# Carlos310197/Fast-Point-Cloud-Registration-with-GPUs

Measured on AMD Instinct MI355X. Metric: ICP iterations/sec + NN HBM GB/s (% roofline), hall cloud, higher is better.
Workload: dtype f32

## Files before the change

fast-point-cloud-registration-with-gpus_amd/csrc/icp_device_sparse.h:

```cpp
#pragma once
#include "icp_device.h"

namespace icp {

template <bool HIER> struct SpHit { using type = unsigned short; };
template <> struct SpHit<true> { using type = int; };

constexpr bool SP_XY_EARLY_OUT = false;

template <bool PERM, int S>
__device__ __forceinline__ void scan_hit_half(const float* sb, int ch, const f2 px, const f2 py, const f2 pz, float& best, int& bj, float (&bq)[3])
{
    constexpr int C = 8;
    const float *qxp = sb + 8, *qyp = sb + 16, *qzp = sb + 24;
    const float4 qxa = *reinterpret_cast<const float4*>(qxp), qxb = *reinterpret_cast<const float4*>(qxp + 4);
    const float4 qya = *reinterpret_cast<const float4*>(qyp), qyb = *reinterpret_cast<const float4*>(qyp + 4);
    const float4 qza = *reinterpret_cast<const float4*>(qzp), qzb = *reinterpret_cast<const float4*>(qzp + 4);
    f2 d[C / 2];
    {
        f2 ax, ay, az;
        ax = pk_sub_sel<S>(f2{qxa.x, qxa.y}, px); ay = pk_sub_sel<S>(f2{qya.x, qya.y}, py); az = pk_sub_sel<S>(f2{qza.x, qza.y}, pz); d[0] = (ax * ax + ay * ay) + az * az;
        ax = pk_sub_sel<S>(f2{qxa.z, qxa.w}, px); ay = pk_sub_sel<S>(f2{qya.z, qya.w}, py); az = pk_sub_sel<S>(f2{qza.z, qza.w}, pz); d[1] = (ax * ax + ay * ay) + az * az;
        ax = pk_sub_sel<S>(f2{qxb.x, qxb.y}, px); ay = pk_sub_sel<S>(f2{qyb.x, qyb.y}, py); az = pk_sub_sel<S>(f2{qzb.x, qzb.y}, pz); d[2] = (ax * ax + ay * ay) + az * az;
        ax = pk_sub_sel<S>(f2{qxb.z, qxb.w}, px); ay = pk_sub_sel<S>(f2{qyb.z, qyb.w}, py); az = pk_sub_sel<S>(f2{qzb.z, qzb.w}, pz); d[3] = (ax * ax + ay * ay) + az * az;
    }
    float c0 = fmin_(fmin_(d[0].x, d[0].y), fmin_(d[1].x, d[1].y));
    c0 = fmin_(c0, fmin_(fmin_(d[2].x, d[2].y), fmin_(d[3].x, d[3].y)));
    auto dk = [&](int k) { return (k & 1) ? d[k >> 1].y : d[k >> 1].x; };
    if constexpr (PERM) {
        const bool cand = c0 <= best;
        if (__builtin_amdgcn_ballot_w64(cand) != 0ull) {
            const int* qo = reinterpret_cast<const int*>(sb + 32);
            int o0 = 0x7fffffff, k0 = 0;
#pragma unroll
            for (int kk = C - 1; kk >= 0; --kk) {
                const int oj = qo[kk];
                const bool e0 = (dk(kk) == c0) & (oj < o0);
                o0 = e0 ? oj : o0; k0 = e0 ? kk : k0;
            }
            const bool take = cand & ((c0 < best) | (bj < 0) | (o0 < bj));
            best = take ? c0 : best;
            bj = take ? o0 : bj;
            if (take) { bq[0] = qxp[k0]; bq[1] = qyp[k0]; bq[2] = qzp[k0]; }
        }
    } else {
        const bool take = (c0 < best) | ((c0 == best) & (ch < (bj >> 3)));
        if (__builtin_amdgcn_ballot_w64(take) != 0ull) {
            int k0 = C - 1;
#pragma unroll
            for (int kk = C - 2; kk >= 0; --kk) k0 = (dk(kk) == c0) ? kk : k0;
            best = take ? c0 : best;
            bj = take ? ch * C + k0 : bj;
            if (take) { bq[0] = qxp[k0]; bq[1] = qyp[k0]; bq[2] = qzp[k0]; }
        }
    }
}

template <bool PERM, bool HALVES = false>
__device__ __forceinline__ int scan_hit(const float* sb, int ch, const f2 px, const f2 py, const f2 pz, float (&best)[2], int (&bj)[2],
                                        float (&bq)[2][3])
{
    constexpr int C = 8;
    {
        if constexpr (HALVES) {
            const f2 gx = px - f2{__builtin_amdgcn_fmed3f(px.x, sb[0], sb[3]), __builtin_amdgcn_fmed3f(px.y, sb[0], sb[3])};
            const f2 gy = py - f2{__builtin_amdgcn_fmed3f(py.x, sb[1], sb[4]), __builtin_amdgcn_fmed3f(py.y, sb[1], sb[4])};
            const f2 gz = pz - f2{__builtin_amdgcn_fmed3f(pz.x, sb[2], sb[5]), __builtin_amdgcn_fmed3f(pz.y, sb[2], sb[5])};
            f2 L = (gx * gx + gy * gy) + gz * gz;
            L = L * f2{0.99999905f, 0.99999905f};
            const unsigned long long m0 = __builtin_amdgcn_ballot_w64(L.x <= best[0]), m1 = __builtin_amdgcn_ballot_w64(L.y <= best[1]);
            if ((m0 | m1) == 0ull) return 0;
            if (m1 == 0ull) { scan_hit_half<PERM, 0>(sb, ch, px, py, pz, best[0], bj[0], bq[0]); return 2; }
            if (m0 == 0ull) { scan_hit_half<PERM, 1>(sb, ch, px, py, pz, best[1], bj[1], bq[1]); return 2; }
        } else {
        const f2 pxa[1] = {px}, pya[1] = {py}, pza[1] = {pz};
        if (__builtin_amdgcn_ballot_w64(box_may_improve<1, true>(sb[0], sb[1], sb[2], sb[3], sb[4], sb[5], pxa, pya, pza, best)) == 0ull) return 0;
        }
    }
    const float *qxp = sb + 8, *qyp = sb + 16, *qzp = sb + 24;
    f2 d[C];
    float mxy0 = inf_<float>(), mxy1 = inf_<float>();
#pragma unroll
    for (int kk = 0; kk < C; kk += 4) {
        const float4 qx4 = *reinterpret_cast<const float4*>(qxp + kk);
        const float4 qy4 = *reinterpret_cast<const float4*>(qyp + kk);
        const f2 qxa = f2{qx4.x, qx4.y}, qxb = f2{qx4.z, qx4.w};
        const f2 qya = f2{qy4.x, qy4.y}, qyb = f2{qy4.z, qy4.w};
        f2 ax, ay;
        ax = pk_sub_bcast<0>(qxa, px); ay = pk_sub_bcast<0>(qya, py);
        d[kk + 0] = ax * ax + ay * ay;
        ax = pk_sub_bcast<1>(qxa, px); ay = pk_sub_bcast<1>(qya, py);
        d[kk + 1] = ax * ax + ay * ay;
        ax = pk_sub_bcast<0>(qxb, px); ay = pk_sub_bcast<0>(qyb, py);
        d[kk + 2] = ax * ax + ay * ay;
        ax = pk_sub_bcast<1>(qxb, px); ay = pk_sub_bcast<1>(qyb, py);
        d[kk + 3] = ax * ax + ay * ay;
        if constexpr (SP_XY_EARLY_OUT) {
            mxy0 = fmin_(fmin_(mxy0, d[kk].x), d[kk + 1].x);
            mxy0 = fmin_(fmin_(mxy0, d[kk + 2].x), d[kk + 3].x);
            mxy1 = fmin_(fmin_(mxy1, d[kk].y), d[kk + 1].y);
            mxy1 = fmin_(fmin_(mxy1, d[kk + 2].y), d[kk + 3].y);
        }
    }
    if constexpr (SP_XY_EARLY_OUT) {
        if (__builtin_amdgcn_ballot_w64((mxy0 <= best[0]) | (mxy1 <= best[1])) == 0ull) return 1;
    }
    float c0 = inf_<float>(), c1 = inf_<float>();
#pragma unroll
    for (int kk = 0; kk < C; kk += 4) {
        const float4 qz4 = *reinterpret_cast<const float4*>(qzp + kk);
        const f2 qza = f2{qz4.x, qz4.y}, qzb = f2{qz4.z, qz4.w};
        f2 az;
        az = pk_sub_bcast<0>(qza, pz); d[kk + 0] = d[kk + 0] + az * az;
        az = pk_sub_bcast<1>(qza, pz); d[kk + 1] = d[kk + 1] + az * az;
        az = pk_sub_bcast<0>(qzb, pz); d[kk + 2] = d[kk + 2] + az * az;
        az = pk_sub_bcast<1>(qzb, pz); d[kk + 3] = d[kk + 3] + az * az;
        c0 = fmin_(fmin_(c0, d[kk].x), d[kk + 1].x);
        c0 = fmin_(fmin_(c0, d[kk + 2].x), d[kk + 3].x);
        c1 = fmin_(fmin_(c1, d[kk].y), d[kk + 1].y);
        c1 = fmin_(fmin_(c1, d[kk + 2].y), d[kk + 3].y);
    }
    if constexpr (PERM) {
        const bool cand0 = c0 <= best[0], cand1 = c1 <= best[1];
        if (__builtin_amdgcn_ballot_w64(cand0 | cand1) != 0ull) {
            const int* qo = reinterpret_cast<const int*>(sb + 32);
            int o0 = 0x7fffffff, o1 = 0x7fffffff, k0 = 0, k1 = 0;
// ... 283 lines not shown
```

fast-point-cloud-registration-with-gpus_amd/csrc/icp_k_sparse.hip:

```cpp
#include "icp_device_sparse.h"
#include <math.h>
#include <stdlib.h>
#include <cstring>

namespace icp {


template <int TAIL, bool DIAG, bool PERM, bool HIER = false, int NWS = SP_NW>
__global__ __launch_bounds__(NWS * 64, NWS == 16 ? 1 : 4) void nn_match_sparse(const float* __restrict__ P, int n_pad,
                                                              const float* __restrict__ Q, int m_pad, int seg_len,
                                                              int round_passes, float* __restrict__ part_d,
                                                              int32_t* __restrict__ part_idx, RT<float> rt_arg, NNFuse fuse,
                                                              NNTail tail)
{
    constexpr int STG = PERM ? 40 : 32;
    constexpr int SMAX = NWS != 16 ? 1024 : 2048;
    constexpr int HITS_BYTES = SP_HCAP * 4, MQ_BYTES = NWS * 128 * 4;
    constexpr int SUPER_BYTES = HIER ? 2 * NWS * 64 * 4 : 0;
    constexpr int MKEY_OFF = 3 * SMAX * 4 > HITS_BYTES + SUPER_BYTES ? 3 * SMAX * 4 : HITS_BYTES + SUPER_BYTES;
    constexpr int OVL_BYTES = NWS != 16 ? MKEY_OFF + 128 * 8 : HITS_BYTES + 2 * SP_NW * 128 * 4;
    constexpr int TR_BYTES = TAIL ? ((TAIL == 2 ? 28 : 18) * 65 + 64) * 8 : 0;
    static_assert(TR_BYTES <= HITS_BYTES, "the tail's transpose buffer overlays the hit list");
    constexpr int HB = HIER ? 16 : 8;
    constexpr int STAGE_OFF = OVL_BYTES + 128 * 4 + 16, STAGE_BYTES = NWS * HB * STG * 4;
// ... 61 lines not shown
                const unsigned int sums[4] = {s01 & 0xffffu, s01 >> 16, s23 & 0xffffu, s23 >> 16};
                T = share_pick(T0, Tmin, sums, gridDim.x);
            }
            unsigned int S = parts_for(T);
            int v = (int)S;
#pragma unroll
            for (int o = 1; o < 64; o <<= 1) { const int u = __shfl_up(v, o, 64); v += lane >= o ? u : 0; }
            if (lane == 63) role[4 + NWS + w] = v;
            __syncthreads();
            int base = 0;
#pragma unroll
            for (int k = 0; k < NWS; ++k) base += k < w ? role[4 + NWS + k] : 0;
            int all = 0;
#pragma unroll
            for (int k = 0; k < NWS; ++k) all += role[4 + NWS + k];
            const bool fits = all <= (int)gridDim.x;
            const int excl = fits ? base + v - (int)S : t;
            if (!fits) S = t < R ? 1u : 0u;
            if (t < R && (int)blockIdx.x >= excl && (int)blockIdx.x < excl + (int)S) { role[0] = t; role[1] = (int)blockIdx.x - excl; role[2] = (int)S; if constexpr (DIAG) { role[3] = (int)h; role[4] = (int)T; } }
            __syncthreads();
            if (role[0] < 0) return;
            if (t == 0) role[5] = 0;
        }
    }
    if constexpr (HIER && TAIL != 0) {
        if (fuse.row_order != nullptr) {
            int bpos = (int)blockIdx.x;
            {
                const int sh = fuse.xcd_shift, span = 8 << sh;
                if (sh > 0 && bpos < ((int)gridDim.x / span) * span) {
                    const int x = bpos & 7, i = bpos >> 3;
                    bpos = ((((i >> sh) << 3) + x) << sh) + (i & ((1 << sh) - 1));
                }
            }
            const int ro = fuse.row_order[bpos];
            if (ro < 0) return;
            if (threadIdx.x == 0) {
                role[0] = ro & ((1 << NN_ROLE_ROW_BITS) - 1);
                role[1] = (ro >> NN_ROLE_ROW_BITS) & ((1 << NN_ROLE_PART_BITS) - 1);
                role[2] = 1 << ((ro >> (NN_ROLE_ROW_BITS + NN_ROLE_PART_BITS)) & 7);
            }
            __syncthreads();
        }
    }
    unsigned int hsum = 0;
    const int ibase = SP_ROW * 128 + lane;
    int pi[2];
#pragma unroll
    for (int t = 0; t < 2; ++t) pi[t] = fuse.p_perm ? fuse.p_perm[ibase + t * 64] : ibase + t * 64;
    float* stage = reinterpret_cast<float*>(lds_raw + STAGE_OFF) + w * (HB * STG);
    float* msg = reinterpret_cast<float*>(lds_raw + MSG_OFF);
    float (*seedq)[128] = reinterpret_cast<float (*)[128]>(lds_raw + SEED_OFF);
    float (*mq)[NWS][128] = reinterpret_cast<float (*)[NWS][128]>(lds_raw + MQ_OFF);
    int phase_pass_ = 0;
    constexpr int phase_nw_ = NWS;
    constexpr bool phase_diag_ = DIAG;
    ICP_PHASE(0)
    const int q0 = SP_SHARED ? 0 : (int)blockIdx.y * seg_len;
    const int c_lo = q0 / 8, c_hi = min(q0 + seg_len, m_pad) / 8;
    bool real[2], sok[2];
    float sq[2][3];
    const bool from_slots = fuse.slot_state != nullptr && fuse.slot_valid != 0;
#pragma unroll
    for (int t = 0; t < 2; ++t) {
        real[t] = ibase + t * 64 < fuse.n;
        sok[t] = false;
        sq[t][0] = sq[t][1] = sq[t][2] = 0.f;
        if (from_slots) {
            const float* ss = fuse.slot_state + 3 * (size_t)n_pad + (ibase + t * 64);
            sq[t][0] = ss[0]; sq[t][1] = ss[(size_t)n_pad]; sq[t][2] = ss[2 * (size_t)n_pad];
            sok[t] = real[t];
        } else {
            const int i = fresh(pi[t]);
            int j = !real[t] ? -1 : fuse.seed_idx ? fuse.seed_idx[i] : (int)(((long long)i * fuse.m) / fuse.n);
            sok[t] = (unsigned)j < (unsigned)fuse.m;
            j = sok[t] ? j : 0;
            const float* Qg = fuse.Q_gather;
            sq[t][0] = Qg[j]; sq[t][1] = Qg[(size_t)m_pad + j]; sq[t][2] = Qg[2 * (size_t)m_pad + j];
        }
    }
    f2 px, py, pz;
    if (from_slots) {
        const float* ss = fuse.slot_state + (fuse.slot_flip ? 6 * (size_t)n_pad : 0) + ibase;
        px = f2{ss[0], ss[64]};
        py = f2{ss[(size_t)n_pad], ss[(size_t)n_pad + 64]};
        pz = f2{ss[2 * (size_t)n_pad], ss[2 * (size_t)n_pad + 64]};
    } else {
        px = f2{P[pi[0]], P[pi[1]]};
        py = f2{P[(size_t)n_pad + pi[0]], P[(size_t)n_pad + pi[1]]};
        pz = f2{P[2 * (size_t)n_pad + pi[0]], P[2 * (size_t)n_pad + pi[1]]};
    }
    float4 pb0 = float4{0.f, 0.f, 0.f, 0.f}, pb1 = pb0;
    float4 (*boxc)[2][64] = reinterpret_cast<float4 (*)[2][64]>(lds_raw + BOXC_OFF) + w * PRE;
    if constexpr (HIER) {
        const int n2_all = ((m_pad >> 3) + 63) >> 6;
        const int t_lo = c_lo >> 12, t_hi = ((((c_hi + 63) >> 6)) + 63) >> 6;
        const int tidx = t_lo + w * 64 + lane;
        const float4* bp = reinterpret_cast<const float4*>(fuse.boxes + (size_t)m_pad + ((size_t)n2_all + (size_t)(tidx < t_hi ? tidx : t_lo)) * 8);
        pb0 = bp[0];
        pb1 = bp[1];
    } else {
        static_assert(PRE == 2, "two passes are fetched together");
        const int tparts = SP_SHARED ? SP_PARTS : 1, tpart = SP_SHARED ? SP_PART : 0;
        const int ca = c_lo + (w * 64 + lane) * tparts + tpart, cb = ca + NWS * 64 * tparts;
        const float4* bpa = reinterpret_cast<const float4*>(fuse.boxes + (size_t)(ca < c_hi ? ca : 0) * 8);
        const float4* bpb = reinterpret_cast<const float4*>(fuse.boxes + (size_t)(cb < c_hi ? cb : 0) * 8);
        const float4 a0 = bpa[0], a1 = bpa[1], b0 = bpb[0], b1 = bpb[1];
        boxc[0][0][lane] = a0; boxc[0][1][lane] = a1;
        boxc[1][0][lane] = b0; boxc[1][1][lane] = b1;
    }
    unsigned int wk_find = 0, wk_upper = 0, wk_hit[3] = {0, 0, 0}, wk_samp = 0;
    bool spec_valid = false;
    float* spst = reinterpret_cast<float*>(lds_raw + SPST_OFF) + w * 8;
    for (int pass = 0;; ++pass) {
    phase_pass_ = pass;
    double err_row = 0.0;
    RT<float> rt = rt_arg;
    int cmd = fuse.apply ? ICP_CMD_TRANSFORM_MATCH : ICP_CMD_MATCH;
    double row_tag = tail.tag;
    unsigned int row_tag_lo = tail.tag_lo;
    const bool have_seeds = pass > 0 || fuse.seed_idx != nullptr;
    if (w == 0) {
        smin[lane] = 0x7f800000u; smin[lane + 64] = 0x7f800000u;
        mkey[lane] = ~0ull; mkey[lane + 64] = ~0ull;
    }
    if (threadIdx.x == 0) {
        if (HIER || pass == 0) *hcount = 0;
        if constexpr (HIER) { hcount[1] = 0; hcount[2] = 0; }
    }
    if (fuse.mailbox != nullptr) {
        const double want = fuse.want + (double)pass;
        if (w == 0) {
            const bool first = (blockIdx.x == 0 && blockIdx.y == 0) || fuse.relay == nullptr;
            const uint32_t* src = (first ? fuse.mailbox : fuse.relay)->w + (lane & 15);
            const uint32_t want32 = (fuse.want_lo + (uint32_t)pass) | 0x80000000u;
            uint32_t word = 0u;
            bool ok = false;
            const long long give_up = (long long)wall_clock64() + (first ? ICP_MAILBOX_BUDGET_TICKS : 2 * ICP_MAILBOX_BUDGET_TICKS);
            for (unsigned int spins = 1;; ++spins) {
                word = first ? __hip_atomic_load(src, __ATOMIC_RELAXED, __HIP_MEMORY_SCOPE_SYSTEM)
                             : __hip_atomic_load(src, __ATOMIC_RELAXED, __HIP_MEMORY_SCOPE_AGENT);
                ok = (uint32_t)__builtin_amdgcn_readlane((int)word, ICP_MB_TAG0) == want32 &&
                     (uint32_t)__builtin_amdgcn_readlane((int)word, ICP_MB_TAG1) == want32;
                if (ok) break;
                if ((spins & 63u) == 0u && (long long)wall_clock64() > give_up) break;
                __builtin_amdgcn_s_sleep(2);
            }
            if (!ok) word = (lane & 15) == ICP_MB_CMD ? (uint32_t)ICP_CMD_EXIT : ((lane & 15) == ICP_MB_TAG0 || (lane & 15) == ICP_MB_TAG1) ? want32 : 0u;
            if (first && fuse.relay != nullptr && lane < 16)
                __hip_atomic_store(&fuse.relay->w[lane], word, __ATOMIC_RELAXED, __HIP_MEMORY_SCOPE_AGENT);
            if (lane < 16) reinterpret_cast<uint32_t*>(msg)[lane] = word;
            if constexpr (!HIER && TAIL != 0) {
                if (pass > 0 && fuse.share_prev != nullptr && role[5] != 0) {
                    const float* pub = fuse.seed_pub + (size_t)SP_ROW * 384;
#pragma unroll
                    for (int a = 0; a < 3; ++a) {
                        seedq[a][lane] = __hip_atomic_load(&pub[a * 128 + lane], __ATOMIC_RELAXED, __HIP_MEMORY_SCOPE_AGENT);
                        seedq[a][lane + 64] = __hip_atomic_load(&pub[a * 128 + lane + 64], __ATOMIC_RELAXED, __HIP_MEMORY_SCOPE_AGENT);
                    }
                }
            }
        }
        __syncthreads();
        cmd = reinterpret_cast<const int*>(msg)[ICP_MB_CMD];
// ... 161 lines not shown
        const float gz = __builtin_fmaxf(__builtin_fmaxf(b0.z - gh[2], gl[2] - b1.y), 0.f);
        const float L = ((gx * gx + gy * gy) + gz * gz) * 0.99999905f;
        const bool pass = cidx < c_hi && L < B;
        if constexpr (DIAG) wk_find += (unsigned int)__builtin_popcountll(__builtin_amdgcn_ballot_w64(cidx < c_hi));
        const unsigned long long mask = __builtin_amdgcn_ballot_w64(pass);
        if (mask != 0ull) {
            int base = 0;
            if (lane == 0) base = atomicAdd(hcount, (int)__builtin_popcountll(mask));
            base = __builtin_amdgcn_readfirstlane(base);
            const int rank = __builtin_amdgcn_mbcnt_hi((unsigned)(mask >> 32), __builtin_amdgcn_mbcnt_lo((unsigned)mask, 0));
            if (pass) hits[base + rank] = (hit_t)cidx;
        }
    };
    auto gather_batch = [&](const int hb, const int h1) {
            {
                const int part = lane & 7;
                const int r0 = lane >> 3, h0 = hb + r0 * NWS + w, h8 = hb + (r0 + 8) * NWS + w;
                const bool on0 = h0 < h1, on8 = HB > 8 && h8 < h1;
                const int ch0 = on0 ? (int)hits[h0] : 0, ch8 = on8 ? (int)hits[h8] : 0;
                const float* src0 = HIER ? fuse.records + (size_t)ch0 * NN_REC_WORDS + part * 4
                                         : part < 2 ? fuse.boxes + (size_t)ch0 * 8 + part * 4 : Q + (size_t)((part - 2) >> 1) * m_pad + (size_t)ch0 * 8 + (part & 1) * 4;
                const float* src8 = HIER ? fuse.records + (size_t)ch8 * NN_REC_WORDS + part * 4
                                         : part < 2 ? fuse.boxes + (size_t)ch8 * 8 + part * 4 : Q + (size_t)((part - 2) >> 1) * m_pad + (size_t)ch8 * 8 + (part & 1) * 4;
                float4 v0 = float4{0.f, 0.f, 0.f, 0.f}, v8 = v0;
                if (on0) v0 = *reinterpret_cast<const float4*>(src0);
                if constexpr (HB > 8) { if (on8) v8 = *reinterpret_cast<const float4*>(src8); }
                if (on0) *reinterpret_cast<float4*>(stage + r0 * STG + part * 4) = v0;
                if constexpr (HB > 8) { if (on8) *reinterpret_cast<float4*>(stage + (r0 + 8) * STG + part * 4) = v8; }
                if constexpr (PERM) {
                    const int r2 = lane >> 1, half = lane & 1;
                    const int h2 = hb + r2 * NWS + w;
                    if (lane < 2 * HB && h2 < h1)
                        *reinterpret_cast<int4*>(stage + r2 * STG + 32 + half * 4) =
                            HIER ? *reinterpret_cast<const int4*>(fuse.records + (size_t)(int)hits[h2] * NN_REC_WORDS + 32 + half * 4)
                                 : *reinterpret_cast<const int4*>(fuse.q_perm + (size_t)(int)hits[h2] * 8 + half * 4);
                }
            }
            lds_same_wave_order();
    };
    auto scan_batch = [&](const int hb, const int h1) {
            const int mine = (h1 - hb - w + NWS - 1) / NWS;
            const int cnt = mine < HB ? mine : HB;
            const bool share_minima = h1 > NWS * HB;
            if (share_minima && hb != 0) {
#pragma unroll
                for (int t = 0; t < 2; ++t) {
                    const unsigned int v = smin[lane + t * 64];
                    if (real[t] && v < 0x7f800000u && v < __float_as_uint(best[t])) { best[t] = __uint_as_float(v + 1u); bj[t] = -1; }
                }
            }
            for (int rr = 0; rr < cnt; ++rr) {
                int stage_reached;
                if constexpr (PERM) {
                    stage_reached = scan_hit<true, true>(stage + rr * STG, 0, px, py, pz, best, bj, bq);
                } else {
                    const int ch = __builtin_amdgcn_readfirstlane((int)hits[hb + rr * NWS + w]);
                    stage_reached = scan_hit<false, true>(stage + rr * STG, ch, px, py, pz, best, bj, bq);
                }
                if constexpr (DIAG) {
                    ++wk_hit[0];
                    wk_hit[1] += stage_reached >= 1 ? 1u : 0u;
                    wk_hit[2] += stage_reached >= 2 ? 1u : 0u;
                }
            }
            if (share_minima && hb + NWS * HB < h1) {
                if (real[0] && bj[0] >= 0) atomicMin(&smin[lane], __float_as_uint(best[0]));
                if (real[1] && bj[1] >= 0) atomicMin(&smin[lane + 64], __float_as_uint(best[1]));
            }
            lds_same_wave_order();
    };
    auto sub_stamp = [&](int k) {
        if constexpr (DIAG && !HIER) {
            if (fuse.tlog != nullptr && w == 2 && lane == 0 && (fuse.tlog_pass < 0 || fuse.tlog_pass == phase_pass_)) {
                const long long slot_ = (((long long)blockIdx.y * gridDim.x + blockIdx.x) * phase_nw_ + w) * 10 + k;
                if (slot_ < fuse.tlog_cap) fuse.tlog[slot_] = (long long)wall_clock64();
            }
        }
    };
    auto process_hits = [&](const int h1) {
        for (int hb = 0; hb < h1; hb += NWS * HB) {
            gather_batch(hb, h1);
            if (hb == 0) sub_stamp(7);
            scan_batch(hb, h1);
        }
    };
    auto exchange = [&]() {
        if (real[0]) atomicMin(&smin[lane], __float_as_uint(best[0]));
        if (real[1]) atomicMin(&smin[lane + 64], __float_as_uint(best[1]));
        __syncthreads();
        if (threadIdx.x == 0) *hcount = 0;
#pragma unroll
        for (int t = 0; t < 2; ++t) {
            const unsigned int v = smin[lane + t * 64];
            if (real[t] && v < 0x7f800000u && v < __float_as_uint(best[t])) { best[t] = __uint_as_float(v + 1u); bj[t] = -1; }
        }
    };
    auto find_round = [&](int tb, float B, const float (&gl)[3], const float (&gh)[3]) {
        const int tparts = SP_SHARED ? SP_PARTS : 1, tpart = SP_SHARED ? SP_PART : 0;
        int r = 0;
        if (tb == 0) {
#pragma unroll
            for (; r < PRE; ++r) {
                const int cidx = c_lo + ((r * NWS + w) * 64 + lane) * tparts + tpart;
                if constexpr (!HIER)
                    if (r < round_passes && c_lo + ((r * NWS + w) * 64) * tparts + tpart < c_hi) find_pass(cidx, boxc[r][0][lane], boxc[r][1][lane], B, gl, gh);
            }
        }
        for (; r < round_passes; r += 4) {
            int cidx[4];
            float4 b0[4], b1[4];
#pragma unroll
            for (int q = 0; q < 4; ++q) {
                cidx[q] = c_lo + ((tb + (r + q) * NWS + w) * 64 + lane) * tparts + tpart;
                const bool on = r + q < round_passes && cidx[q] < c_hi;
                const float4* bp = reinterpret_cast<const float4*>(fuse.boxes + (size_t)(on ? cidx[q] : c_lo) * 8);
// ... 154 lines not shown
        if constexpr (DIAG) {
            if (fuse.work != nullptr && threadIdx.x == 0) {
                atomicAdd(&fuse.work[NN_WORK_SPEC_LISTS], 1ull);
                if (covered) { atomicAdd(&fuse.work[NN_WORK_SPEC_COVERED], 1ull); atomicAdd(&fuse.work[NN_WORK_SPEC_HITS], (unsigned long long)*hcount); }
            }
        }
        if (covered) {
            const int h1 = *hcount;
            scan_batch(0, h1);
            for (int hb = NWS * HB; hb < h1; hb += NWS * HB) { gather_batch(hb, h1); scan_batch(hb, h1); }
            searched = true;
        } else {
            if (threadIdx.x == 0) *hcount = 0;
            __syncthreads();
        }
    }
    if (!searched) {
    for (int tb = 0; tb < own_tiles; tb += round_tiles) {
        const float B = tb == 0 ? B0 : wave_minmax<true>(__builtin_fmaxf(best[0], best[1]));
        if (tb != 0) __syncthreads();
        find_round(tb, B, glo, ghi);
        __syncthreads();
        if (tb == 0) sub_stamp(6);
        if (SP_SHARED && threadIdx.x == 0) {
            __hip_atomic_fetch_add(&fuse.share_cur[SP_ROW], (unsigned int)*hcount, __ATOMIC_RELAXED, __HIP_MEMORY_SCOPE_AGENT);
            if (fuse.share_cur2 != nullptr) __hip_atomic_fetch_add(&fuse.share_cur2[SP_ROW], (unsigned int)*hcount, __ATOMIC_RELAXED, __HIP_MEMORY_SCOPE_AGENT);
        }
        if constexpr (DIAG) {
            if (fuse.tlog != nullptr && w == 1 && lane == 0 && (fuse.tlog_pass < 0 || fuse.tlog_pass == phase_pass_)) {
                const long long slot_ = (((long long)blockIdx.y * gridDim.x + blockIdx.x) * phase_nw_ + w) * 10;
                if (slot_ + 9 < fuse.tlog_cap) {
                    fuse.tlog[slot_ + 6] = ((long long)SP_ROW << 32) | ((long long)SP_PART << 16) | (long long)SP_PARTS;
                    fuse.tlog[slot_ + 7] = (tb == 0 ? 0ll : fuse.tlog[slot_ + 7]) + (long long)*hcount;
                    if (SP_SHARED) fuse.tlog[slot_ + 8] = ((long long)role[4] << 32) | (long long)(unsigned int)role[3];
                }
            }
        }
        if constexpr (DIAG) { if (fuse.work != nullptr && threadIdx.x == 0) atomicAdd(&fuse.work[NN_WORK_LIST_HITS], (unsigned long long)*hcount); }
        process_hits(*hcount);
        if (tb + round_tiles < own_tiles) exchange();
    }
    }
    spec_valid = false;
    }
    ICP_PHASE(3)
    if constexpr (DIAG) {
        if (fuse.work != nullptr && lane == 0) {
            if (wk_find) atomicAdd(&fuse.work[NN_WORK_FIND_BOXES], (unsigned long long)wk_find);
            if (wk_upper) atomicAdd(&fuse.work[NN_WORK_UPPER_BOXES], (unsigned long long)wk_upper);
            if (wk_hit[0]) atomicAdd(&fuse.work[NN_WORK_HITS_BOX], (unsigned long long)wk_hit[0]);
            if (wk_hit[1]) atomicAdd(&fuse.work[NN_WORK_HITS_XY], (unsigned long long)wk_hit[1]);
            if (wk_hit[2]) atomicAdd(&fuse.work[NN_WORK_HITS_FULL], (unsigned long long)wk_hit[2]);
            if (wk_samp) atomicAdd(&fuse.work[NN_WORK_SAMPLE_GROUPS], (unsigned long long)wk_samp);
            if (w == 0) atomicAdd(&fuse.work[NN_WORK_BLOCK_PASSES], 1ull);
            if (w == 0 && apply) atomicAdd(&fuse.work[NN_WORK_BLOCK_TRANSFORMS], 1ull);
        }
        wk_find = wk_upper = wk_samp = 0; wk_hit[0] = wk_hit[1] = wk_hit[2] = 0;
    }

    if (SP_ORDERED && threadIdx.x == 0 && hsum != 0u) __hip_atomic_fetch_add(&fuse.row_hits[SP_ROW], hsum, __ATOMIC_RELAXED, __HIP_MEMORY_SCOPE_AGENT);
#pragma unroll
    for (int t = 0; t < 2; ++t) {
        if (bj[t] >= 0) {
            const unsigned long long key = ((unsigned long long)__float_as_uint(best[t]) << 32) | ((unsigned int)bj[t] << 4) | (unsigned int)w;
            atomicMin(&mkey[lane + t * 64], key);
            mq[0][w][lane + t * 64] = bq[t][0]; mq[1][w][lane + t * 64] = bq[t][1]; mq[2][w][lane + t * 64] = bq[t][2];
        }
    }
    if (w == 0) {
        const bool none0 = real[0] && best[0] == inf_<float>(), none1 = real[1] && best[1] == inf_<float>();
        if (__builtin_amdgcn_ballot_w64(none0 | none1) != 0ull) {
            const float* Qg = fuse.Q_gather;
            const float q0x = Qg[0], q0y = Qg[(size_t)m_pad], q0z = Qg[2 * (size_t)m_pad];
            if (none0) { atomicMin(&mkey[lane], (unsigned long long)0x7f800000u << 32); mq[0][0][lane] = q0x; mq[1][0][lane] = q0y; mq[2][0][lane] = q0z; }
            if (none1) { atomicMin(&mkey[lane + 64], (unsigned long long)0x7f800000u << 32); mq[0][0][lane + 64] = q0x; mq[1][0][lane + 64] = q0y; mq[2][0][lane + 64] = q0z; }
        }
    }
    ICP_PHASE(4)
    __syncthreads();
    ICP_PHASE(5)
    if (w != 0) {
        if (!fuse.resident) return;
    } else {
    float fb[2];
    int fj[2];
#pragma unroll
    for (int t = 0; t < 2; ++t) {
        const unsigned long long key = mkey[lane + t * 64];
        const bool none = key == ~0ull;
        const unsigned int lo = (unsigned int)key;
        fb[t] = none ? inf_<float>() : __uint_as_float((unsigned int)(key >> 32));
        fj[t] = none ? 0x7fffffff : (int)(lo >> 4);
        const int bw = none ? 0 : (int)(lo & 15u);
        sq[t][0] = mq[0][bw][lane + t * 64]; sq[t][1] = mq[1][bw][lane + t * 64]; sq[t][2] = mq[2][bw][lane + t * 64];
    }
    if constexpr (TAIL == 0) {
#pragma unroll
        for (int t = 0; t < 2; ++t) {
            const size_t o = (size_t)blockIdx.y * n_pad + (size_t)pi[t];
            part_d[o] = fb[t];
            part_idx[o] = fj[t];
        }
        return;
    } else {
        const int parts = SP_PARTS, row = SP_ROW;
        bool closer = true;
        if (parts > 1) {
#pragma unroll
            for (int t = 0; t < 2; ++t) {
                const unsigned long long key = ((unsigned long long)__float_as_uint(fb[t]) << 32) | (unsigned int)fj[t];
// ... 138 lines not shown
```

fast-point-cloud-registration-with-gpus_amd/csrc/icp_kernels.h:

```cpp
#pragma once
#include <hip/hip_runtime.h>
#include <cstdint>
#include <stdint.h>

#include "../../include/icp_mi355x.h"
#include "icp_plan.h"

namespace icp {

#if defined(__HIPCC__)
#define ICP_HOST_DEVICE __host__ __device__
#else
#define ICP_HOST_DEVICE
#endif
struct alignas(64) NNMailbox {
    uint32_t w[16];
};
enum { ICP_MB_TAG0 = 7, ICP_MB_CMD = 13, ICP_MB_TAG1 = 14 };
ICP_HOST_DEVICE inline uint32_t mailbox_tag(double seq) { return (uint32_t)(unsigned long long)seq | 0x80000000u; }
ICP_HOST_DEVICE inline int mailbox_rt_word(int k) { return k < 7 ? k : k + 1; }
enum { ICP_CMD_EXIT = 0, ICP_CMD_MATCH = 1, ICP_CMD_TRANSFORM_MATCH = 2, ICP_CMD_TRANSFORM_ONLY = 3 };
struct alignas(128) NNMailbox64 {
    uint32_t w[32];
};
enum { ICP_MB64_CMD = 6 };
#define ICP_MAILBOX_BUDGET_S 4
constexpr long long ICP_MAILBOX_BUDGET_TICKS = (long long)ICP_MAILBOX_BUDGET_S * 100000000ll;
struct NNFusedTransform {
    const double* R9;
    const double* t3;
    const int32_t* idx_prev;
    void* P_out;
    double* err_rows;
    const NNMailbox* mailbox = nullptr;
    NNMailbox* relay = nullptr;
    double want = 0.0;
    bool resident = false;
    bool store_first = false;
    void* slot_state = nullptr;
    bool slot_valid = false;
    bool slot_flip = false;
};

struct NNCullInputs {
    const void* Q_scan;
    const int32_t* seed_idx;
    const void* boxes;
    const void* samples = nullptr;
    int waves64 = 0;
    const NNTuning* tune = nullptr;
    const void* Q_scan_sorted = nullptr;
    const int32_t* q_perm = nullptr;
    const int32_t* p_perm = nullptr;
    unsigned long long* work = nullptr;
    unsigned int* share_counts = nullptr;
    unsigned long long* share_seq = nullptr;
    unsigned long long* share_cold_seq = nullptr;
    float* seed_pub = nullptr;
    const int32_t* row_order = nullptr;
    unsigned int* row_hits = nullptr;
    bool order_history = false;
    const float* records = nullptr;
};
enum {
    NN_WORK_FIND_BOXES = 0,
    NN_WORK_UPPER_BOXES = 1,
    NN_WORK_HITS_BOX = 2,
    NN_WORK_HITS_XY = 3,
    NN_WORK_HITS_FULL = 4,
    NN_WORK_SAMPLE_GROUPS = 5,
    NN_WORK_BLOCK_PASSES = 6,
    NN_WORK_BLOCK_TRANSFORMS = 7,
    NN_WORK_SPEC_LISTS = 8,
    NN_WORK_SPEC_COVERED = 9,
    NN_WORK_SPEC_HITS = 10,
    NN_WORK_LIST_HITS = 11,
    NN_WORK_SLOTS = 12
};
constexpr unsigned int SHARE_COUNT_CLAMP = 1u << 20;
constexpr unsigned int SHARE_MAX_PARTS = 32u;
ICP_HOST_DEVICE inline unsigned int share_clamp(unsigned int h) { return h > SHARE_COUNT_CLAMP ? SHARE_COUNT_CLAMP : h; }
ICP_HOST_DEVICE inline unsigned int share_cap(int m_pad)
{
    const unsigned int tiles = (unsigned int)((((m_pad >> 3) + 63) >> 6));
    return tiles < SHARE_MAX_PARTS ? (tiles < 1u ? 1u : tiles) : SHARE_MAX_PARTS;
}
ICP_HOST_DEVICE inline unsigned int share_parts(unsigned int h, unsigned int T, unsigned int cap)
{
    unsigned int S = (h + T - 1u) / T;
    S = S > cap ? cap : S;
    return S < 1u ? 1u : S;
}
ICP_HOST_DEVICE inline unsigned int share_first_target(unsigned int total, unsigned int spare) { return spare ? (total + spare - 1u) / spare : 0xffffffffu; }
ICP_HOST_DEVICE inline unsigned int share_candidate(unsigned int T0, int k) { return (T0 * (unsigned int)(4 + k) + 7u) / 8u; }
ICP_HOST_DEVICE inline bool share_tries_candidates(unsigned int T0, unsigned int Tmin, unsigned int spare) { return spare != 0u && T0 > Tmin && T0 < 0x10000000u; }
ICP_HOST_DEVICE inline unsigned int share_pick(unsigned int T0, unsigned int Tmin, const unsigned int (&sums)[4], unsigned int blocks)
{
    unsigned int T = T0;
    for (int k = 3; k >= 0; --k) T = sums[k] <= blocks ? share_candidate(T0, k) : T;
    return T < Tmin ? Tmin : T;
}
unsigned int share_rows_plan(const unsigned int* hits, int rows, int blocks, int m_pad, int min_hits, int* parts_out);

constexpr int NN_ORDER_EXTRA = 4096;
constexpr int NN_ORDER_CLASS_BITS = 1;
constexpr int NN_ORDER_XCD_SHIFT = 4;
constexpr int NN_ORDER_HEAD = 1024;
constexpr int NN_REC_WORDS = 40;
size_t model_records_bytes(int m_pad);
hipError_t launch_model_records(const void* Qs_soa, const float* boxes, const int32_t* perm, int m_pad, float* rec, hipStream_t st);

struct RowOrderBuffers {
    unsigned int* keys[2];
    int32_t* vals[2];
    void* temp;
    size_t temp_bytes;
    int32_t* roles;
    unsigned long long* totals;
    unsigned long long seq;
    int min_part;
    int total_div;
    int control = 1;
    int coarse = NN_ORDER_CLASS_BITS;
};
size_t row_order_temp_bytes(int rows);
hipError_t launch_row_order(const RowOrderBuffers& b, unsigned int* hits, int rows, const int32_t** roles_out, hipStream_t st);

struct PrepBuffers {
    unsigned int* keys[2];
    int32_t* vals[2];
// ... 320 lines not shown
```

fast-point-cloud-registration-with-gpus_amd/engine.py:

```python
import ctypes as C
from dataclasses import dataclass, field

import numpy as np

from . import _capi as capi


@dataclass
class Result:
    T: np.ndarray
    iterations: int
    passes: int
    err: np.ndarray
    idx: np.ndarray
    moved: np.ndarray
    seconds_total: float = 0.0
    seconds_nn: float = 0.0
    seconds_host: float = 0.0
    seconds_setup: float = 0.0
    extra: dict = field(default_factory=dict)


def _as_cloud(a, dtype=None):
    a = np.asarray(a)
# ... 79 lines not shown
        return idx

    nn_match = Matching

    def set_model(self, Q):
        Q = _as_cloud(Q)
        capi.check(self._lib.icp_set_model(self._h, Q.ctypes.data, Q.shape[0], _prec(Q.dtype)), "icp_set_model")
        self._dtype, self._m = Q.dtype, Q.shape[0]

    def set_moving(self, P):
        P = _as_cloud(P, self._dtype)
        capi.check(self._lib.icp_set_moving(self._h, P.ctypes.data, P.shape[0], _prec(P.dtype)), "icp_set_moving")
        self._dtype, self._n = P.dtype, P.shape[0]

    def set_model_normals(self, Nrm):
        Nrm = _as_cloud(Nrm, self._dtype)
        capi.check(self._lib.icp_set_model_normals(self._h, Nrm.ctypes.data, Nrm.shape[0]), "icp_set_model_normals")

    def reset_moving(self):
        capi.check(self._lib.icp_reset_moving(self._h), "icp_reset_moving")

    def get_moving(self):
        out = np.empty((self._n, 3), dtype=self._dtype)
        capi.check(self._lib.icp_get_moving(self._h, out.ctypes.data), "icp_get_moving")
        return out

    def get_indices(self):
        out = np.empty(self._n, dtype=np.int32)
        capi.check(self._lib.icp_get_indices(self._h, out.ctypes.data), "icp_get_indices")
        return out

    def nn_match_resident(self, timed=False):
        ms = C.c_float(0)
        capi.check(self._lib.icp_nn_match_resident(self._h, C.byref(ms) if timed else None), "icp_nn_match_resident")
        return ms.value

    def nn_match_bench(self, reps, seeded=True):
        ms = C.c_float(0)
        capi.check(self._lib.icp_nn_match_bench_ex(self._h, int(reps), 1 if seeded else 0, C.byref(ms)), "icp_nn_match_bench_ex")
        return ms.value

    def nn_match_bench_launches(self, reps=10, warmups=2, mode=0):
        out = np.zeros(int(reps), dtype=np.float32)
        capi.check(self._lib.icp_nn_match_bench_launches(self._h, int(reps), int(warmups), int(mode),
                                                         out.ctypes.data_as(C.POINTER(C.c_float))), "icp_nn_match_bench_launches")
        return out

    def nn_launch_info_ex(self, dense=False):
        v = [C.c_int(0) for _ in range(5)]
        capi.check(self._lib.icp_nn_launch_info_ex(self._h, 1 if dense else 0, *[C.byref(x) for x in v]), "icp_nn_launch_info_ex")
        return dict(zip(("splits", "blocks", "threads", "n_pad", "m_pad"), (x.value for x in v)))

    WORK_SLOTS = ("find_boxes", "upper_boxes", "hits_box", "hits_xy", "hits_full", "sample_groups", "block_passes", "block_transforms",
                  "spec_lists", "spec_covered", "spec_hits", "list_hits")

    def set_work_counting(self, enable=True):
        capi.check(self._lib.icp_set_work_counting(self._h, 1 if enable else 0), "icp_set_work_counting")

    def get_work_counters(self, reset=True):
        out = np.zeros(12, dtype=np.uint64)
        capi.check(self._lib.icp_get_work_counters(self._h, out.ctypes.data_as(C.POINTER(C.c_uint64)), 1 if reset else 0),
                   "icp_get_work_counters")
        return dict(zip(self.WORK_SLOTS, (int(x) for x in out)))

    def diag_row_roles(self, hits, min_part=2048, total_div=4096, control=True):
        h = np.ascontiguousarray(hits, dtype=np.uint32).copy()
        roles = np.zeros(h.size + 4096, dtype=np.int32)
        capi.check(self._lib.icp_diag_row_roles(self._h, h.ctypes.data_as(C.POINTER(C.c_uint32)), int(h.size), int(min_part), int(total_div), 1 if control else 0,
                                                roles.ctypes.data_as(C.POINTER(C.c_int32))), "icp_diag_row_roles")
        return roles, h

    def diag_loop_moments(self):
        mom = np.zeros(capi.ICP_NMOM, dtype=np.float64)
        route = C.c_int(0)
        capi.check(self._lib.icp_diag_loop_moments(self._h, mom.ctypes.data_as(C.POINTER(C.c_double)), C.byref(route)), "icp_diag_loop_moments")
        return mom, route.value

    def nn_launch_info(self):
        v = [C.c_int(0) for _ in range(5)]
        capi.check(self._lib.icp_nn_launch_info(self._h, *[C.byref(x) for x in v]), "icp_nn_launch_info")
        return dict(zip(("splits", "blocks", "threads", "n_pad", "m_pad"), (x.value for x in v)))

    def estimate_normals(self, want_neighbours=False):
        nrm = np.empty((self._m, 3), dtype=self._dtype)
        nbr = np.empty((self._m, 4), dtype=np.int32) if want_neighbours else None
        capi.check(self._lib.icp_estimate_normals(self._h, nrm.ctypes.data, nbr.ctypes.data if want_neighbours else None),
                   "icp_estimate_normals")
        return (nrm, nbr) if want_neighbours else nrm

    def _run(self, metric, D, M, normals, max_iter, tol, fixed_iterations):
        D = _as_cloud(D)
        M = _as_cloud(M, D.dtype)
        n, m = D.shape[0], M.shape[0]
        prm = capi.icp_params(int(max_iter), float(tol), 1 if fixed_iterations else 0, _prec(D.dtype), metric)
        err = np.zeros(int(max_iter) + 1, dtype=np.float64)
        idx = np.zeros(n, dtype=np.int32)
        moved = np.zeros((n, 3), dtype=D.dtype)
        res = capi.icp_result()
        res.err = err.ctypes.data_as(C.POINTER(C.c_double))
        res.idx = idx.ctypes.data_as(C.POINTER(C.c_int32))
        res.moved = moved.ctypes.data
        if metric == capi.ICP_POINT_TO_PLANE:
            nptr = None
            if normals is not None:
                normals = _as_cloud(normals, D.dtype)
                nptr = normals.ctypes.data
            rc = self._lib.icp_point_to_plane(self._h, D.ctypes.data, n, M.ctypes.data, m, nptr, C.byref(prm), C.byref(res))
            capi.check(rc, "icp_point_to_plane")
        else:
            rc = self._lib.icp_point_to_point(self._h, D.ctypes.data, n, M.ctypes.data, m, C.byref(prm), C.byref(res))
            capi.check(rc, "icp_point_to_point")
        self._dtype, self._n, self._m = D.dtype, n, m
        return Result(T=np.array(res.T[:], dtype=np.float64).reshape(4, 4), iterations=res.iterations,
# ... 1078 lines not shown
```

include/icp_mi355x_diag.h:

```cpp
#ifndef ICP_MI355X_DIAG_H
#define ICP_MI355X_DIAG_H

#include "icp_mi355x.h"

#ifdef __cplusplus
extern "C" {
#endif

int icp_nn_match_bench(icp_ctx* ctx, int reps, float* total_ms);
int icp_nn_match_bench_ex(icp_ctx* ctx, int reps, int seeded, float* total_ms);
int icp_nn_match_bench_launches(icp_ctx* ctx, int reps, int warmups, int mode, float* each_ms);
int icp_nn_launch_info_ex(icp_ctx* ctx, int dense, int* splits, int* blocks, int* threads, int* n_pad, int* m_pad);
#define ICP_WORK_SLOTS 12
int icp_set_work_counting(icp_ctx* ctx, int enable);
int icp_get_work_counters(icp_ctx* ctx, uint64_t* out_slots, int reset);

int icp_share_rows_plan(const uint32_t* hits, int rows, int blocks, int model_points, int min_hits, int32_t* parts, uint32_t* target);
#define ICP_ROLES_EXTRA 4096
int icp_diag_row_roles(icp_ctx* ctx, uint32_t* hits_io, int rows, int min_part, int total_div, int control, int32_t* roles_out);

#define ICP_ROUTE_HOST_ROWS 0x001
#define ICP_ROUTE_COMPACT 0x002
#define ICP_ROUTE_AVX 0x004
#define ICP_ROUTE_FIN_LAUNCH 0x008
#define ICP_ROUTE_FIN_PINNED 0x010
#define ICP_ROUTE_FIN_KERNEL 0x020
#define ICP_ROUTE_FIN_TWO_STAGE 0x040
#define ICP_ROUTE_FUSED_TAIL 0x080
#define ICP_ROUTE_MOMENTS_KERNEL 0x100
#define ICP_ROUTE_ERROR_ONLY 0x200
#define ICP_ROUTE_ARMED 0x400
#define ICP_ROUTE_RESIDENT 0x800
int icp_diag_loop_moments(icp_ctx* ctx, double* out32, int* route);
int icp_diag_batch_moments(icp_batch* b, int pair, double* out32);
int icp_diag_batch_trim(icp_batch* b, int pair, double* tau_sq, int* rank);
int icp_diag_batch_reverse(icp_batch* b, int32_t* rev_out);
#define ICP_EVAL_SD 0
#define ICP_EVAL_CNT 1
#define ICP_EVAL_SQ 2
#define ICP_EVAL_SQQ 5
int icp_diag_batch_eval_moments(icp_batch* b, int pair, double* out32);
int icp_diag_batch_rotation(icp_batch* b, int pair, double* R9);

int icp_diag_batch_set_features(icp_batch* b, const double* moving_feat, const double* model_feat);
int icp_diag_batch_ransac(icp_batch* b, int pair, int32_t* triples, uint8_t* valid, double* T16, int32_t* counts);
int icp_diag_batch_fgr(icp_batch* b, int pair, int32_t* used_pos, double* mu_hist, double* mom_hist, double* T_hist);
int icp_diag_batch_fgr_times(icp_batch* b, double* seconds4);
#ifdef __cplusplus
}
#endif
#endif
```

Measured before the change: 113,900.

## Fold both query halves into one lane-compacted scan when few lanes ask

Adds a fold path to the sparse NN hit scan. When both per-lane query halves have candidates but together they need at most 64 lanes, the second-half queries are moved through LDS (via mbcnt lane ranking) into lanes whose first half does not need the hit. The chunk is then scanned once instead of twice and the results are routed back. This cuts the double 8-point distance evaluation on mixed hits, at the cost of extra LDS traffic, more registers and some divergent select logic. A diagnostic counter for folded hits is also added.

```diff
diff --git a/fast-point-cloud-registration-with-gpus_amd/csrc/icp_device_sparse.h b/fast-point-cloud-registration-with-gpus_amd/csrc/icp_device_sparse.h
--- a/fast-point-cloud-registration-with-gpus_amd/csrc/icp_device_sparse.h
+++ b/fast-point-cloud-registration-with-gpus_amd/csrc/icp_device_sparse.h
@@ -56,10 +56,91 @@
     }
 }
 
-template <bool PERM, bool HALVES = false>
+template <bool PERM>
+__device__ __forceinline__ void scan_hit_fold(const float* sb, int ch, const f2 px, const f2 py, const f2 pz, float (&best)[2], int (&bj)[2],
+                                              float (&bq)[2][3], const bool keep, const bool lend, const unsigned long long m0,
+                                              const unsigned long long m1, f2* fa, f2* fb)
+{
+    constexpr int C = 8;
+    const unsigned long long mf = ~m0;
+    const int j = (int)__builtin_amdgcn_mbcnt_hi((unsigned)(m1 >> 32), __builtin_amdgcn_mbcnt_lo((unsigned)m1, 0));
+    const int r = (int)__builtin_amdgcn_mbcnt_hi((unsigned)(mf >> 32), __builtin_amdgcn_mbcnt_lo((unsigned)mf, 0));
+    const bool borrow = !keep & (r < (int)__builtin_popcountll(m1));
+    const float *qxp = sb + 8, *qyp = sb + 16, *qzp = sb + 24;
+    const float4 qxa = *reinterpret_cast<const float4*>(qxp), qxb = *reinterpret_cast<const float4*>(qxp + 4);
+    const float4 qya = *reinterpret_cast<const float4*>(qyp), qyb = *reinterpret_cast<const float4*>(qyp + 4);
+    const float4 qza = *reinterpret_cast<const float4*>(qzp), qzb = *reinterpret_cast<const float4*>(qzp + 4);
+    if (lend) { fa[j] = f2{px.y, py.y}; fb[j] = f2{pz.y, best[1]}; }
+    asm volatile("" ::: "memory");
+    const f2 ga = fa[r], gb = fb[r];
+    const f2 pxy = f2{keep ? px.x : ga.x, keep ? py.x : ga.y};
+    const f2 pzb = f2{keep ? pz.x : gb.x, keep ? best[0] : borrow ? gb.y : -1.f};
+    f2 d[C / 2];
+    {
+        f2 ax, ay, az;
+        ax = pk_sub_sel<0>(f2{qxa.x, qxa.y}, pxy); ay = pk_sub_sel<1>(f2{qya.x, qya.y}, pxy); az = pk_sub_sel<0>(f2{qza.x, qza.y}, pzb); d[0] = (ax * ax + ay * ay) + az * az;
+        ax = pk_sub_sel<0>(f2{qxa.z, qxa.w}, pxy); ay = pk_sub_sel<1>(f2{qya.z, qya.w}, pxy); az = pk_sub_sel<0>(f2{qza.z, qza.w}, pzb); d[1] = (ax * ax + ay * ay) + az * az;
+        ax = pk_sub_sel<0>(f2{qxb.x, qxb.y}, pxy); ay = pk_sub_sel<1>(f2{qyb.x, qyb.y}, pxy); az = pk_sub_sel<0>(f2{qzb.x, qzb.y}, pzb); d[2] = (ax * ax + ay * ay) + az * az;
+        ax = pk_sub_sel<0>(f2{qxb.z, qxb.w}, pxy); ay = pk_sub_sel<1>(f2{qyb.z, qyb.w}, pxy); az = pk_sub_sel<0>(f2{qzb.z, qzb.w}, pzb); d[3] = (ax * ax + ay * ay) + az * az;
+    }
+    float c0 = fmin_(fmin_(d[0].x, d[0].y), fmin_(d[1].x, d[1].y));
+    c0 = fmin_(c0, fmin_(fmin_(d[2].x, d[2].y), fmin_(d[3].x, d[3].y)));
+    auto dk = [&](int k) { return (k & 1) ? d[k >> 1].y : d[k >> 1].x; };
+    if (__builtin_amdgcn_ballot_w64(c0 <= pzb.y) == 0ull) return;
+    int word;
+    if constexpr (PERM) {
+        const int* qo = reinterpret_cast<const int*>(sb + 32);
+        int o0 = 0x7fffffff, k0 = 0;
+#pragma unroll
+        for (int kk = C - 1; kk >= 0; --kk) {
+            const int oj = qo[kk];
+            const bool e0 = (dk(kk) == c0) & (oj < o0);
+            o0 = e0 ? oj : o0; k0 = e0 ? kk : k0;
+        }
+        word = (int)(((unsigned int)o0 << 3) | (unsigned int)k0);
+    } else {
+        int k0 = C - 1;
+#pragma unroll
+        for (int kk = C - 2; kk >= 0; --kk) k0 = (dk(kk) == c0) ? kk : k0;
+        word = k0;
+    }
+    if (borrow) fa[r] = f2{c0, __int_as_float(word)};
+    asm volatile("" ::: "memory");
+    const f2 back = fa[j];
+    const float c[2] = {c0, back.x};
+    const int wd[2] = {word, __float_as_int(back.y)};
+    const bool asked[2] = {keep, lend};
+#pragma unroll
+    for (int t = 0; t < 2; ++t) {
+        const int k0 = wd[t] & 7;
+        bool take;
+        int nj;
+        if constexpr (PERM) {
+            nj = (int)((unsigned int)wd[t] >> 3);
+            take = asked[t] & (c[t] <= best[t]) & ((c[t] < best[t]) | (bj[t] < 0) | (nj < bj[t]));
+        } else {
+            nj = ch * C + k0;
+            take = asked[t] & ((c[t] < best[t]) | ((c[t] == best[t]) & (ch < (bj[t] >> 3))));
+        }
+        best[t] = take ? c[t] : best[t];
+        bj[t] = take ? nj : bj[t];
+        if (take) { bq[t][0] = qxp[k0]; bq[t][1] = qyp[k0]; bq[t][2] = qzp[k0]; }
+    }
+}
+
+#ifndef SP_FOLD_MAX
+#define SP_FOLD_MAX 64
+#endif
+constexpr bool sp_fold_form(int tail, bool perm, bool hier, int nws)
+{
+    return tail == 2 ? false : tail == 0 ? true : nws == 16 ? perm != hier : perm || hier;
+}
+
+template <bool PERM, bool HALVES = false, int FOLD = 0>
 __device__ __forceinline__ int scan_hit(const float* sb, int ch, const f2 px, const f2 py, const f2 pz, float (&best)[2], int (&bj)[2],
-                                        float (&bq)[2][3])
-{
+                                        float (&bq)[2][3], f2* fa = nullptr, f2* fb = nullptr)
+{
+    static_assert(FOLD >= 0 && FOLD <= 64 && (FOLD == 0 || HALVES), "one lane per asking slot");
     constexpr int C = 8;
     {
         if constexpr (HALVES) {
@@ -72,6 +153,12 @@
             if ((m0 | m1) == 0ull) return 0;
             if (m1 == 0ull) { scan_hit_half<PERM, 0>(sb, ch, px, py, pz, best[0], bj[0], bq[0]); return 2; }
             if (m0 == 0ull) { scan_hit_half<PERM, 1>(sb, ch, px, py, pz, best[1], bj[1], bq[1]); return 2; }
+            if constexpr (FOLD > 0) {
+                if ((int)__builtin_popcountll(m0) + (int)__builtin_popcountll(m1) <= FOLD) {
+                    scan_hit_fold<PERM>(sb, ch, px, py, pz, best, bj, bq, L.x <= best[0], L.y <= best[1], m0, m1, fa, fb);
+                    return 3;
+                }
+            }
         } else {
         const f2 pxa[1] = {px}, pya[1] = {py}, pza[1] = {pz};
         if (__builtin_amdgcn_ballot_w64(box_may_improve<1, true>(sb[0], sb[1], sb[2], sb[3], sb[4], sb[5], pxa, pya, pza, best)) == 0ull) return 0;
diff --git a/fast-point-cloud-registration-with-gpus_amd/csrc/icp_k_sparse.hip b/fast-point-cloud-registration-with-gpus_amd/csrc/icp_k_sparse.hip
--- a/fast-point-cloud-registration-with-gpus_amd/csrc/icp_k_sparse.hip
+++ b/fast-point-cloud-registration-with-gpus_amd/csrc/icp_k_sparse.hip
@@ -137,6 +137,9 @@
     float* msg = reinterpret_cast<float*>(lds_raw + MSG_OFF);
     float (*seedq)[128] = reinterpret_cast<float (*)[128]>(lds_raw + SEED_OFF);
     float (*mq)[NWS][128] = reinterpret_cast<float (*)[NWS][128]>(lds_raw + MQ_OFF);
+    constexpr int FOLD = sp_fold_form(TAIL, PERM, HIER, NWS) ? SP_FOLD_MAX : 0;
+    f2* const fold_a = reinterpret_cast<f2*>(&mq[0][w][0]);
+    f2* const fold_b = reinterpret_cast<f2*>(&mq[1][w][0]);
     int phase_pass_ = 0;
     constexpr int phase_nw_ = NWS;
     constexpr bool phase_diag_ = DIAG;
@@ -194,7 +197,7 @@
         boxc[0][0][lane] = a0; boxc[0][1][lane] = a1;
         boxc[1][0][lane] = b0; boxc[1][1][lane] = b1;
     }
-    unsigned int wk_find = 0, wk_upper = 0, wk_hit[3] = {0, 0, 0}, wk_samp = 0;
+    unsigned int wk_find = 0, wk_upper = 0, wk_hit[3] = {0, 0, 0}, wk_samp = 0, wk_fold = 0;
     bool spec_valid = false;
     float* spst = reinterpret_cast<float*>(lds_raw + SPST_OFF) + w * 8;
     for (int pass = 0;; ++pass) {
@@ -462,15 +465,16 @@
             for (int rr = 0; rr < cnt; ++rr) {
                 int stage_reached;
                 if constexpr (PERM) {
-                    stage_reached = scan_hit<true, true>(stage + rr * STG, 0, px, py, pz, best, bj, bq);
+                    stage_reached = scan_hit<true, true, FOLD>(stage + rr * STG, 0, px, py, pz, best, bj, bq, fold_a, fold_b);
                 } else {
                     const int ch = __builtin_amdgcn_readfirstlane((int)hits[hb + rr * NWS + w]);
-                    stage_reached = scan_hit<false, true>(stage + rr * STG, ch, px, py, pz, best, bj, bq);
+                    stage_reached = scan_hit<false, true, FOLD>(stage + rr * STG, ch, px, py, pz, best, bj, bq, fold_a, fold_b);
                 }
                 if constexpr (DIAG) {
                     ++wk_hit[0];
                     wk_hit[1] += stage_reached >= 1 ? 1u : 0u;
                     wk_hit[2] += stage_reached >= 2 ? 1u : 0u;
+                    wk_fold += stage_reached == 3 ? 1u : 0u;
                 }
             }
             if (share_minima && hb + NWS * HB < h1) {
@@ -731,10 +735,11 @@
             if (wk_hit[1]) atomicAdd(&fuse.work[NN_WORK_HITS_XY], (unsigned long long)wk_hit[1]);
             if (wk_hit[2]) atomicAdd(&fuse.work[NN_WORK_HITS_FULL], (unsigned long long)wk_hit[2]);
             if (wk_samp) atomicAdd(&fuse.work[NN_WORK_SAMPLE_GROUPS], (unsigned long long)wk_samp);
+            if (wk_fold) atomicAdd(&fuse.work[NN_WORK_HITS_FOLDED], (unsigned long long)wk_fold);
             if (w == 0) atomicAdd(&fuse.work[NN_WORK_BLOCK_PASSES], 1ull);
             if (w == 0 && apply) atomicAdd(&fuse.work[NN_WORK_BLOCK_TRANSFORMS], 1ull);
         }
-        wk_find = wk_upper = wk_samp = 0; wk_hit[0] = wk_hit[1] = wk_hit[2] = 0;
+        wk_find = wk_upper = wk_samp = wk_fold = 0; wk_hit[0] = wk_hit[1] = wk_hit[2] = 0;
     }
 
     if (SP_ORDERED && threadIdx.x == 0 && hsum != 0u) __hip_atomic_fetch_add(&fuse.row_hits[SP_ROW], hsum, __ATOMIC_RELAXED, __HIP_MEMORY_SCOPE_AGENT);
diff --git a/fast-point-cloud-registration-with-gpus_amd/csrc/icp_kernels.h b/fast-point-cloud-registration-with-gpus_amd/csrc/icp_kernels.h
--- a/fast-point-cloud-registration-with-gpus_amd/csrc/icp_kernels.h
+++ b/fast-point-cloud-registration-with-gpus_amd/csrc/icp_kernels.h
@@ -75,7 +75,8 @@
     NN_WORK_SPEC_COVERED = 9,
     NN_WORK_SPEC_HITS = 10,
     NN_WORK_LIST_HITS = 11,
-    NN_WORK_SLOTS = 12
+    NN_WORK_HITS_FOLDED = 12,
+    NN_WORK_SLOTS = 13
 };
 constexpr unsigned int SHARE_COUNT_CLAMP = 1u << 20;
 constexpr unsigned int SHARE_MAX_PARTS = 32u;
diff --git a/fast-point-cloud-registration-with-gpus_amd/engine.py b/fast-point-cloud-registration-with-gpus_amd/engine.py
--- a/fast-point-cloud-registration-with-gpus_amd/engine.py
+++ b/fast-point-cloud-registration-with-gpus_amd/engine.py
@@ -155,13 +155,13 @@
         return dict(zip(("splits", "blocks", "threads", "n_pad", "m_pad"), (x.value for x in v)))
 
     WORK_SLOTS = ("find_boxes", "upper_boxes", "hits_box", "hits_xy", "hits_full", "sample_groups", "block_passes", "block_transforms",
-                  "spec_lists", "spec_covered", "spec_hits", "list_hits")
+                  "spec_lists", "spec_covered", "spec_hits", "list_hits", "hits_folded")
 
     def set_work_counting(self, enable=True):
         capi.check(self._lib.icp_set_work_counting(self._h, 1 if enable else 0), "icp_set_work_counting")
 
     def get_work_counters(self, reset=True):
-        out = np.zeros(12, dtype=np.uint64)
+        out = np.zeros(len(self.WORK_SLOTS), dtype=np.uint64)
         capi.check(self._lib.icp_get_work_counters(self._h, out.ctypes.data_as(C.POINTER(C.c_uint64)), 1 if reset else 0),
                    "icp_get_work_counters")
         return dict(zip(self.WORK_SLOTS, (int(x) for x in out)))
diff --git a/include/icp_mi355x_diag.h b/include/icp_mi355x_diag.h
--- a/include/icp_mi355x_diag.h
+++ b/include/icp_mi355x_diag.h
@@ -11,7 +11,7 @@
 int icp_nn_match_bench_ex(icp_ctx* ctx, int reps, int seeded, float* total_ms);
 int icp_nn_match_bench_launches(icp_ctx* ctx, int reps, int warmups, int mode, float* each_ms);
 int icp_nn_launch_info_ex(icp_ctx* ctx, int dense, int* splits, int* blocks, int* threads, int* n_pad, int* m_pad);
-#define ICP_WORK_SLOTS 12
+#define ICP_WORK_SLOTS 13
 int icp_set_work_counting(icp_ctx* ctx, int enable);
 int icp_get_work_counters(icp_ctx* ctx, uint64_t* out_slots, int reset);
 
```

Measured after the change: 106,500. 0.935x the previous value.
